# yinyunie/Pose2Room

Measured on AMD Instinct MI355X. Metric: P2RNet train-step samples/sec (T=1024,J=53,bs=32), higher is better.
Workload: dtype f32; 1 GPU; P2RNet full train step, bs=32/GPU, T=1024, J=53, seeds=512, proposals=128 (BASELINE configs[2]); input=P2RNet_dataloader over SyntheticPoseDataset, global_batch=32, frames=1024, parallelism=dp1

## Files before the change

include/p2r_hip.h:

```cpp
#ifndef P2R_HIP_H
#define P2R_HIP_H

#include <stdint.h>

#ifdef __cplusplus
extern "C" {
#endif

#define P2R_OK 0
#define P2R_EINVAL (-22)

int p2r_abi_version(void);
const char *p2r_build_arch(void);


int p2r_furthest_point_sampling(int b, int n, int m, const float *dataset,
                                float *temp, int *idxs, void *stream);

int p2r_gather_points(int b, int c, int n, int npoints, const float *points,
                      const int *idx, float *out, void *stream);

int p2r_gather_points_grad(int b, int c, int n, int npoints,
                           const float *grad_out, const int *idx,
                           float *grad_points, void *stream);

int p2r_ball_query(int b, int n, int m, float radius, int nsample,
                   const float *new_xyz, const float *xyz, int *idx,
                   void *stream);

int p2r_group_points(int b, int c, int n, int npoints, int nsample,
                     const float *points, const int *idx, float *out,
                     void *stream);

int p2r_group_points_grad(int b, int c, int n, int npoints, int nsample,
                          const float *grad_out, const int *idx,
                          float *grad_points, void *stream);

int p2r_three_nn(int b, int n, int m, const float *unknown, const float *known,
                 float *dist2, int *idx, void *stream);

int p2r_three_interpolate(int b, int c, int m, int n, const float *points,
                          const int *idx, const float *weight, float *out,
                          void *stream);

int p2r_three_interpolate_grad(int b, int c, int n, int m,
                               const float *grad_out, const int *idx,
                               const float *weight, float *grad_points,
                               void *stream);


#define P2R_NND_L2 0
#define P2R_NND_L1SMOOTH 1
#define P2R_NND_L1 2

int p2r_nn_distance(int B, int N, int M, int C, const float *pc1,
                    const float *pc2, int mode, float delta, float *dist1,
                    int64_t *idx1, float *dist2, int64_t *idx2, void *stream);

int p2r_nn_distance_grad(int B, int N, int M, int C, const float *pc1,
                         const float *pc2, int mode, float delta,
                         const int64_t *idx1, const int64_t *idx2,
                         const float *g1, const float *g2, float *grad_pc1,
                         float *grad_pc2, void *stream);


int p2r_det_loss_forward(int B, int S, int J, int T, int K, int G, int NC, int j0, float near_thr,
                         float far_thr, float w0, float w1, const float *seed_skeleton,
                         const float *vote_xyz, const int64_t *seed_inds, const float *vote_label,
                         const int64_t *vote_label_mask, const float *agg_xyz, const float *center,
                         const float *size, const double *heading, const float *obj_scores,
                         const float *sem_scores, const float *center_label, const float *box_mask,
                         const float *gt_size, const float *gt_heading, const int64_t *gt_cls,
                         float *partial, double *partial64, float *out32, double *out64, float *g_vote,
                         float *g_obj, float *g_c1, float *g_c2, float *g_size, double *g_head,
                         float *g_sem, void *stream);

int p2r_det_loss_backward(int B, int S, int K, int NC, const double *coef, const float *out32,
                          const float *g_vote, const float *g_obj, const float *g_c1, const float *g_c2,
                          const float *g_size, const double *g_head, const float *g_sem, float *d_vote,
                          float *d_obj, float *d_center, float *d_size, double *d_head, float *d_sem,
                          void *stream);


int p2r_nms3d(int B, int K, int stride, const double *boxes,
              const uint8_t *valid, double overlap_threshold, int old_type,
              int same_cls, uint8_t *keep, int *pick, int *npick, void *stream);


int p2r_stgcn_gcn_forward(int N, int T, int V, int K, const int *Lk_host,
                          const float *x, const float *W, const uint8_t *nbr,
                          const float *coef, const float *bias_cv, float *z,
                          float *stats_partial, void *stream);

int p2r_stgcn_gcn2_forward(int N, int T, int V, int K, int ltot, const float *x, const float *Wp,
                           const float *coef, const int *stream, int *stream_work,
                           const float *bias_cv, const float *addend, float *z, float *stats_partial,
                           int *n_partials, const float *bwd_u, const unsigned char *bwd_mask,
                           const float *bwd_fin, void *stream_h);

unsigned long long p2r_stgcn_gcn3_signature(int form);
int p2r_stgcn_gcn3_forward(int N, int T, int V, int K, int ltot, int form, const float *x, const float *Wp,
                           const float *coef, const float *bias_cv, const float *addend, float *z,
                           float *stats_partial, int *n_partials, const float *bwd_u,
                           const unsigned char *bwd_mask, const float *bwd_fin, void *stream_h);

int p2r_stgcn_gcn3_data_gradient_masked_addend(int N, int T, int V, int K, int ltot, const float *x,
                                               const float *Wp, const float *coef, const float *addend,
                                               const unsigned char *addend_mask, float *z, float *stats_partial,
                                               const float *bwd_u, const unsigned char *bwd_mask,
                                               const float *bwd_fin, void *stream_h);

int p2r_stgcn_gcn3_coef_grad(int N, int T, int V, int K, int ltot, const float *x, const float *dz,
                             const float *Wp, int n_blocks, float *dcoef_partial, void *stream);

int p2r_stgcn_gcn3_weight_grad(int N, int T, int V, int K, int ltot, const float *x, const float *dz,
                               const float *coef, int n_blocks, float *dw_partial, float *colsum_partial,
                               void *stream);

int p2r_stgcn_gcn_weight_grad(int N, int T, int V, int K, const int *Lk_host,
                              const float *x, const float *dz,
                              const uint8_t *nbr, const float *coef,
                              int n_blocks, float *dw_partial, float *colsum_partial,
                              int colsum_of_x, void *stream);

int p2r_stgcn_gcn_coef_grad(int N, int T, int V, int K, const int *Lk_host,
                            const float *x, const float *dz, const float *Wt,
                            const uint8_t *nbr, const float *coef, int n_blocks,
                            float *dcoef_partial, void *stream);


int p2r_bn_stats(int rows, int L, const float *x, float *partial, void *stream);

int p2r_bn_apply(int N, int C, int L, const float *x, const float *scale,
                 const float *shift, const float *res, int relu, float *y,
                 unsigned char *relu_mask, void *stream);

int p2r_bn_bwd_reduce(int N, int C, int L, const float *dy, const float *y,
                      const float *x, const float *mean, const float *invstd,
                      int relu, const float *mscale, const float *mshift,
                      float *partial, void *stream);

int p2r_bn_bwd_apply(int N, int C, int L, const float *dy, const float *y,
                     const float *x, const float *mean, const float *invstd,
                     const float *kscale, const float *m1, const float *m2,
                     int relu, const float *mscale, const float *mshift,
                     float *dx, float *dres, void *stream);

int p2r_bn_finalize(int P, int C, int width, const float *partial, double M, const float *gamma,
                    const float *beta, double eps, double momentum, float *running_mean,
                    float *running_var, long long *num_batches_tracked, float *out, void *stream);

int p2r_bn_bwd_finalize(int P, int C, const float *partial, double M, float *out, void *stream);


int p2r_stgcn_tconv_forward(int N, int T, int V, int taps, const float *x, const float *scale,
                            const float *shift, const float *W, const float *bias,
                            float *out, float *stats_partial, int *n_partials, void *stream);

int p2r_stgcn_tconv_weight_grad(int N, int T, int V, int taps, const float *x, const float *scale,
                                const float *shift, const float *dout, int n_blocks,
                                float *dw_partial, float *dbias_partial, void *stream);

int p2r_stgcn_tconv_weight_grad_dz(int N, int T, int V, int taps, const float *x, const float *fin,
                                   const float *dout, const float *dh, const float *m12, float *dz, int n_blocks,
                                   float *dw_partial, float *dbias_partial, void *stream);

int p2r_stgcn_tconv2_forward(int N, int T, int V, int taps, const float *x, const float *scale, const float *shift,
                             const float *Wp, const float *bias, float *out, float *stats_partial,
                             int *n_partials, const float *bwd_z, const float *bwd_fin, void *stream);

int p2r_stgcn_tconv3_forward(int N, int T, int V, int taps, const float *x, const float *scale, const float *shift,
                             const float *Wp, const float *bias, float *out, float *stats_partial,
                             int *n_partials, const float *bwd_z, const float *bwd_fin, void *stream);

int p2r_stgcn_tconv3_forward_add(int N, int T, int V, const float *x, const float *scale, const float *shift,
                                 const float *Wp, const float *bias, const float *add_ct, float *out, void *stream);


int p2r_embed3_forward(int N, int L, const float *x, const float *W, const float *bias,
                       float *out, void *stream);

int p2r_embed3_forward_stats(int N, int L, const float *x, const float *W, const float *bias,
                             float *out, float *scratch, float *stats, void *stream);

int p2r_embed3_weight_grad(int N, int L, const float *x, const float *dout, float *partial,
                           void *stream);

int p2r_embed3_weight_grad_lazy(int N, int L, const float *x, const float *g, const float *z, const float *coef,
                                float *partial, void *stream);

int p2r_embed_layer_backward(int N, int L, const float *g, const float *z, const float *coef, const float *zp,
                             const float *fin, const float *W, float *g_prev, float *sums, int n_blocks,
                             float *dw_part, float *db_part, void *stream);

int p2r_colsum(int rows, int T, int V, const float *x, float *out_partial, void *stream);

int p2r_sum_leading(int P, long long M, const float *in, float *out, int tr64, void *stream);


int p2r_sa_votes_forward(int b, int n, int m, int nsample, float radius, int C0,
                         int C1, int C2, const float *xyz, const float *new_xyz,
                         const float *features, const float *w1, const float *b1,
                         const float *w2, const float *b2, int *idx, float *out,
                         float *G, float *H, unsigned char *amax, void *stream);

int p2r_sa_votes_backward(int b, int m, int nsample, int C, const float *dout, const float *out,
                          const unsigned char *amax, const float *H, const float *w2t,
                          const float *w1t, float *dZ2, float *dZ1, float *dG, void *stream);

int p2r_gemm_nt_256(int nb, int L, int split, const float *A, const float *B, float *partial,
                    void *stream);


#define P2R_PW_MAX_JOBS 8

typedef struct p2r_pw_job {
  const float *x, *x2, *tr, *w, *bias, *mz, *mfin;
  float *out, *stats;
  int k, rows, x_ctot, x_nlc, tr_mode, tr_ld, w_t, out_ctot, out_nlc, epilogue, mz_ctot, mfin_ld;
} p2r_pw_job;

int p2r_pw_gemm(int njobs, const p2r_pw_job *jobs, int B, int L, void *stream);

typedef struct p2r_pw_wjob {
  const float *x, *x2, *tr, *y, *ytr;
  float *dw_part, *db_part;
  int rows, k, x_ctot, x_nlc, tr_mode, tr_ld, y_ctot, y_nlc, ytr_ld, split;
} p2r_pw_wjob;
int p2r_pw_wgrad(int njobs, const p2r_pw_wjob *jobs, int B, int L, void *stream);

typedef struct p2r_pw_bnjob {
  const float *part, *gamma, *beta;
  float *running_mean, *running_var, *fin;
  long long *num_batches_tracked;
  double eps, momentum;
  int P, C, fin_ld;
} p2r_pw_bnjob;
int p2r_pw_bn_finalize(int njobs, const p2r_pw_bnjob *jobs, void *stream);

typedef struct p2r_pw_bnbjob {
  const float *part, *fin;
  float *coef, *dgamma, *dbeta;
  double M;
  int P, C, fin_ld, coef_ld, train;
} p2r_pw_bnbjob;
int p2r_pw_bn_bwd_finalize(int njobs, const p2r_pw_bnbjob *jobs, void *stream);

typedef struct p2r_pw_rjob {
  const float *in;
  float *out;
  int P, M;
} p2r_pw_rjob;
#define P2R_PW_MAX_RJOBS 48
int p2r_pw_reduce(int njobs, const p2r_pw_rjob *jobs, void *stream);

typedef struct p2r_mix_head {
  const float *logit, *log_sigma;
  const void *mu, *eps, *dpred;
  void *pred, *dmu;
  float *pi, *dlogit, *dlog_sigma;
  int D, f64;
} p2r_mix_head;
#define P2R_MIX_MAX_HEADS 4
int p2r_mdn_mix_forward(int nheads, const p2r_mix_head *heads, int B, int G, int L, int logit_ctot, void *stream);
int p2r_mdn_mix_backward(int nheads, const p2r_mix_head *heads, int B, int G, int L, int logit_ctot, int dlogit_ctot,
                         void *stream);

typedef struct p2r_mdn_sample_head {
  const float *pi, *log_sigma;
  const void *mu;
  void *out;
  int D, f64, head_id;
} p2r_mdn_sample_head;
#define P2R_MDN_SAMPLE_MAX_HEADS 3
int p2r_mdn_sample(int nheads, const p2r_mdn_sample_head *heads, int B, int G, int L, int pi_ctot, int H,
                   const int *n_samples, unsigned long long seed, int h_offset, void *stream);

typedef struct p2r_sample_store {
  const float *joints, *votes;
  const long long *frame_offset;
  const int *n_frames;
  const double *floor_height, *box_center;
  const float *box_heading, *box_size, *box_mask;
  const long long *box_cls;
  long long n_frames_total;
  int n_samples, J, K;
} p2r_sample_store;
typedef struct p2r_batch_out {
  float *input_joints, *vote_label;
  long long *vote_label_mask;
  float *center_label, *size, *heading, *box_label_mask;
  long long *sem_cls_label;
} p2r_batch_out;
#define P2R_BOX_VARIANTS 9
int p2r_assemble_batch(const p2r_sample_store *store, int B, const long long *sel, const double *aug, int augment,
                       int use_height, int num_frames, const p2r_batch_out *out, void *stream);


int p2r_gather_frames(int b, int c, int t, int j, int s, const float *x, const long long *inds, float *out,
                      void *stream);
int p2r_gather_frames_grad(int b, int c, int t, int j, int s, const float *dout, const long long *inds, float *dx,
                           void *stream);
int p2r_rowsum_short(long long rows, int v_len, float scale, const float *x, float *out, void *stream);

int p2r_vote_finish(int b, int s, int C, const float *net, const float *seed_features, const float *hip,
                    float *vote_xyz, float *feat_ncl, float *inv_norm, void *stream);
int p2r_vote_finish_grad(int b, int s, int C, const float *d_xyz, const float *d_feat, const float *feat_ncl,
                         const float *inv_norm, float *d_net, float *d_sf, void *stream);

int p2r_nearest_prefix(int b, int t, int s, const float *cum, const float *target, long long *inds, void *stream);


int p2r_absmax_bits(long long n, const float *x, unsigned *amax_bits, void *stream);

int p2r_bn_bwd_apply_amax(int N, int C, int L, const float *dy, const unsigned char *mask, const float *x,
                          const float *mean, const float *invstd, const float *kscale, const float *m1,
                          const float *m2, float *dx, float *dres, unsigned *amax_bits, void *stream);
int p2r_bn_apply_amax(int N, int C, int L, const float *x, const float *scale, const float *shift, const float *res,
                      float *y, unsigned char *mask, unsigned *amax_bits, void *stream);
int p2r_stgcn_tconv_weight_grad_dz_amax(int N, int T, int V, int taps, const float *x, const float *fin,
                                        const float *dout, const float *dh, const float *m12, float *dz, int n_blocks,
                                        float *dw_partial, float *dbias_partial, unsigned *amax_bits, void *stream);

int p2r_stgcn_tconvh_forward(int N, int T, int V, const float *x, const float *scale, const float *shift,
                             const void *Wh, const float *winv, const float *bias, float *out, float *stats_partial,
                             int *n_partials, const float *bwd_z, const float *bwd_fin, const unsigned *x_amax,
                             void *stream);

unsigned long long p2r_stgcn_gcn3h_signature(int form);
int p2r_stgcn_gcn3h_pairs(int form, int *pairs);
int p2r_stgcn_gcn3h_forward(int N, int T, int V, int K, int ltot, const float *x, const void *Wh, const float *winv,
                            const float *coef, const float *bias_cv, float *z, float *stats_partial, int *n_partials,
                            const unsigned *x_amax, void *stream);
int p2r_stgcn_gcn3h_data_gradient(int N, int T, int V, int K, int ltot, const float *dz, const void *Wh,
                                  const float *winv, const float *coef, const float *addend,
                                  const unsigned char *addend_mask, float *dx, const unsigned *dz_amax, void *stream);

unsigned long long p2r_stgcn_gcn3h_weight_grad_signature(void);
int p2r_stgcn_gcn3h_weight_grad(int N, int T, int V, int K, int ltot, const float *x, const float *dz, const float *coef,
                                int n_blocks, float *dw_partial, float *dbias_partial, const unsigned *x_amax,
                                const unsigned *dz_amax, void *stream);

int p2r_stgcn_gcn3h_coef_grad(int N, int T, int V, int K, int ltot, const float *x, const float *dz, const void *Wd,
                              const float *winv, int n_blocks, float *dcoef_partial, const unsigned *x_amax,
                              void *stream);

#ifdef __cplusplus
}
#endif
#endif
```

pose2room_amd/p2rnet/modules/stgcn.py:

```python
import torch
import torch.nn as nn

from ..registers import MODULES
from .stgcn_layers import Graph, st_gcn_block
from .sub_modules import SingleConv


def _point_mlp(cin, width, cout):
    return nn.Sequential(SingleConv(cin, width, kernel_size=1, order='cbr', padding=0, ndim=1),
                         SingleConv(width, width, kernel_size=1, order='cbr', padding=0, ndim=1),
                         SingleConv(width, cout, kernel_size=1, order='c', padding=0, ndim=1))


@MODULES.register_module
class STGCN(nn.Module):
    def __init__(self, cfg, optim_spec=None):
        super().__init__()
        self.optim_spec = optim_spec

        self.graph = Graph(layout='virtualroom', strategy='spatial', max_hop=5)
        self.register_buffer('A', torch.tensor(self.graph.A, dtype=torch.float32, requires_grad=False))

        self.n_seeds = cfg.config['data']['num_seeds']
        self.origin_joint_id = cfg.dataset_config.origin_joint_id
        width, out_channels = 64, 256
        kernel_size = (3, self.A.size(0))
        self.knn = 20

        self.pos_embed = _point_mlp(3, 64, width)
        self.sk_feat = _point_mlp(3, 64, width)
        self.st_gcn_networks = nn.ModuleList(
            [st_gcn_block(width, 64, kernel_size, 1, residual=False)] +
            [st_gcn_block(64, 64, kernel_size, 1) for _ in range(5)])
        from ..gcn_op import GraphTables
        tables = GraphTables(self.graph.A)
        for i, blk in enumerate(self.st_gcn_networks):
            blk.gcn.tables = tables
            blk.chain_input = i > 0
        self.conv_joint = nn.Conv1d(cfg.dataset_config.joint_num * 64, out_channels, kernel_size=1)
        self.edge_importance = nn.ParameterList(
            [nn.Parameter(torch.ones(self.A.size())) for _ in self.st_gcn_networks])

        n_frames = cfg.config['data']['num_frames']
        if self.n_seeds >= n_frames:
            self.seed_inds = torch.round(torch.linspace(0, n_frames - 1, self.n_seeds)).long()
        else:
            self.seed_sampling = cfg.config['data']['seed_sampling']

    def _select_seeds(self, hip):
        n_batch, n_frames, _ = hip.shape
        device = hip.device
        if self.n_seeds >= n_frames:
            return self.seed_inds.repeat(n_batch, 1).to(device)
        if self.seed_sampling == 'random':
            inds = torch.argsort(torch.rand(size=(n_batch, n_frames)), dim=1)[:, :self.n_seeds]
            return torch.sort(inds, dim=1)[0].to(device)
        if self.seed_sampling == 'uniform':
            step = torch.norm(torch.diff(hip, dim=1), dim=2)
            cum = torch.cumsum(torch.cat([torch.zeros(size=(n_batch, 1), device=device), step], dim=1).double(),
                               dim=1).float()
            stride = cum[:, -1] / (self.n_seeds - 1)
            target = stride.unsqueeze(-1) * torch.arange(self.n_seeds, dtype=torch.float, device=device)
            if cum.is_cuda and cum.dtype == torch.float32 and n_frames <= 40000:
                from .. import seed_op
                return seed_op.nearest_prefix(cum, target)
            return torch.argmin(torch.abs(cum.unsqueeze(-1) - target.unsqueeze(1)), dim=1)
        raise NotImplementedError

    @staticmethod
    def _mlp(seq, x, inner, add_ct=None):
        from .. import bn_op, tconv_op, embed_op
        if embed_op.supported(seq, x, inner, add_ct):
            return embed_op.embed_mlp(seq, x, inner, add_ct)
        s0, s1, s2 = seq
        fused = (x.is_cuda and len(seq) == 3 and hasattr(s0, 'batchnorm') and hasattr(s1, 'batchnorm')
                 and not hasattr(s2, 'batchnorm') and tconv_op.supported_embed3(x, s0.conv)
                 and x.shape[2] % inner == 0 and inner <= 64)
        if fused:
            z0s = None
            if s0.batchnorm.training:
                z, z0s = tconv_op.embed3(x, s0.conv, want_stats=True)
            else:
                z = tconv_op.embed3(x, s0.conv)
            z = z.view(x.shape[0], 64, x.shape[2] // inner, inner)
            fused = tconv_op.supported_pointwise(z, s0.batchnorm, s1.conv) and \
                tconv_op.supported_pointwise(z, s1.batchnorm, s2.conv)
            if fused:
                if s1.batchnorm.training:
                    z, zs = tconv_op.bn_relu_tconv(z, s0.batchnorm, s1.conv, stats=z0s, want_stats=True)
                    z = tconv_op.bn_relu_tconv(z, s1.batchnorm, s2.conv, stats=zs, add_ct=add_ct)
                else:
                    z = tconv_op.bn_relu_tconv(z, s0.batchnorm, s1.conv)
                    z = tconv_op.bn_relu_tconv(z, s1.batchnorm, s2.conv, add_ct=add_ct)
                return z.view(x.shape[0], 64, x.shape[2])
        for stage in seq:
            if x.is_cuda and hasattr(stage, 'batchnorm') and hasattr(stage, 'ReLU') and \
                    bn_op.supported(x, stage.batchnorm):
                x = bn_op.fused_bn_act(stage.conv(x), stage.batchnorm, None, relu=True)
            else:
                x = stage(x)
        if add_ct is not None:
            x = (x.view(x.shape[0], x.shape[1], -1, inner) + add_ct.unsqueeze(-1)).view(x.shape)
        return x

    def embed(self, input_joints):
        n_batch, n_frames, n_joints, _ = input_joints.shape
        device = input_joints.device
        hip = input_joints[:, :, self.origin_joint_id]
        win = torch.arange(n_frames, device=device).unsqueeze(-1) + \
            torch.arange(-self.knn // 2, self.knn // 2, device=device).unsqueeze(0)
        win = win.clamp_(0, n_frames - 1)
        offs = hip[:, win] - hip.unsqueeze(2)
        pe = self._mlp(self.pos_embed, offs.reshape(n_batch, n_frames * self.knn, 3).transpose(1, 2).contiguous(), self.knn)
        from .. import seed_op
        pe = pe.view(n_batch, -1, n_frames, self.knn)
        fused = seed_op.short_rows_supported(pe)
        pe = seed_op.mean_last(pe) if fused else pe.mean(dim=3)
        rel = input_joints - input_joints[:, :, self.origin_joint_id:self.origin_joint_id + 1]
        sk = self._mlp(self.sk_feat, rel.reshape(n_batch, n_frames * n_joints, 3).transpose(1, 2).contiguous(), n_joints,
                       add_ct=pe)
        return sk.view(n_batch, -1, n_frames, n_joints)

    def forward(self, input_joints, end_points=None):
        end_points = {} if end_points is None else end_points
        n_batch, n_frames, n_joints, n_dim = input_joints.size()
        seed_inds = self._select_seeds(input_joints[:, :, self.origin_joint_id])

        x = self.embed(input_joints)
        blocks = self.st_gcn_networks
        tables = blocks[0].gcn.tables
        if tables is not None and tables.gen2 and all(b.chainable(x, self.A) for b in blocks):
            from ..gcn_op import prepare_chain
            for gcn, prep in zip(blocks, prepare_chain(blocks, self.A, self.edge_importance, tables, frames=x.shape[2])):
                x, _ = gcn(x, prep.Aeff, prepared=prep)
        else:
            for gcn, importance in zip(blocks, self.edge_importance):
                x, _ = gcn(x, self.A * importance)

        seed_skeleton = torch.gather(
            input_joints, 1, seed_inds[:, :, None, None].expand(n_batch, self.n_seeds, n_joints, n_dim))
        if self.n_seeds < n_frames:
            from .. import seed_op
            if seed_op.seed_rows_supported(x, seed_inds):
                rows = seed_op.seed_rows(x, seed_inds)
            else:
                rows = x.permute(0, 2, 1, 3)[torch.arange(n_batch, device=x.device)[:, None], seed_inds]
            seed_features = torch.nn.functional.linear(
                rows.reshape(n_batch, self.n_seeds, -1),
                self.conv_joint.weight.squeeze(-1), self.conv_joint.bias)
        else:
            x = x.transpose(2, 3).reshape(n_batch, -1, n_frames)
            seed_features = self.conv_joint(x).transpose(1, 2)
            seed_features = torch.gather(
                seed_features, 1, seed_inds.unsqueeze(-1).expand(n_batch, self.n_seeds, seed_features.size(-1)))
        end_points['seed_inds'] = seed_inds
        end_points['seed_skeleton'] = seed_skeleton[..., :3]
        end_points['seed_features'] = seed_features
        return end_points
```

pose2room_amd/p2rnet/modules/stgcn_layers.py:

```python
from collections import deque

import numpy as np
import torch
import torch.nn as nn

_VIRTUALROOM_BONES = [
    (0, 1), (1, 3), (3, 5), (5, 19), (0, 2), (2, 4), (4, 6), (6, 20), (0, 7), (7, 8), (8, 9),
    (9, 10), (10, 21), (10, 22), (8, 11), (11, 13), (13, 15), (15, 17), (8, 12), (12, 14),
    (14, 16), (16, 18), (17, 23), (23, 24), (24, 25), (17, 26), (26, 27), (27, 28), (17, 29),
    (29, 30), (30, 31), (17, 32), (32, 33), (33, 34), (17, 35), (35, 36), (36, 37), (18, 38),
    (38, 39), (39, 40), (18, 41), (41, 42), (42, 43), (18, 44), (44, 45), (45, 46), (18, 47),
    (47, 48), (48, 49), (18, 50), (50, 51), (51, 52)]

_LAYOUTS = {'virtualroom': dict(num_node=53, bones=_VIRTUALROOM_BONES, center=0)}


def hop_distance(num_node, edges, max_hop):
    nbr = [[] for _ in range(num_node)]
    for i, j in edges:
        if i != j:
            nbr[i].append(j)
            nbr[j].append(i)
    hop = np.full((num_node, num_node), np.inf)
    for s in range(num_node):
        hop[s, s] = 0
        dq = deque([s])
        while dq:
            u = dq.popleft()
            if hop[s, u] >= max_hop:
                continue
            for v in nbr[u]:
                if np.isinf(hop[s, v]):
                    hop[s, v] = hop[s, u] + 1
                    dq.append(v)
    return hop


class Graph:

    def __init__(self, layout='virtualroom', strategy='spatial', max_hop=5, dilation=1):
        if layout not in _LAYOUTS:
            raise ValueError("Do Not Exist This Layout.")
        spec = _LAYOUTS[layout]
        self.max_hop, self.dilation = max_hop, dilation
        self.num_node, self.center = spec['num_node'], spec['center']
        self.edge = [(i, i) for i in range(self.num_node)] + list(spec['bones'])
        self.hop_dis = hop_distance(self.num_node, self.edge, max_hop)
        self.A = self._adjacency(strategy)

    def _adjacency(self, strategy):
        V = self.num_node
        hops = list(range(0, self.max_hop + 1, self.dilation))
        reach = np.zeros((V, V))
        for h in hops:
            reach[self.hop_dis == h] = 1
        col = reach.sum(0)
        inv = np.zeros(V)
        inv[col > 0] = col[col > 0] ** (-1)
        norm = reach * inv[None, :]
        if strategy == 'uniform':
            return norm[None]
        if strategy == 'distance':
            return np.stack([np.where(self.hop_dis == h, norm, 0.0) for h in hops])
        if strategy == 'spatial':
            dc = self.hop_dis[:, self.center]
            same = dc[:, None] == dc[None, :]
            closer = dc[:, None] > dc[None, :]
            planes = []
            for h in hops:
                at_h = self.hop_dis == h
                root = np.where(at_h & same, norm, 0.0)
                close = np.where(at_h & closer, norm, 0.0)
                further = np.where(at_h & ~same & ~closer, norm, 0.0)
                if h == 0:
                    planes.append(root)
                else:
                    planes.append(root + close)
                    planes.append(further)
            return np.stack(planes)
        raise ValueError("Do Not Exist This Strategy")


class ConvTemporalGraphical(nn.Module):

    def __init__(self, in_channels, out_channels, kernel_size, t_kernel_size=1, t_stride=1,
                 t_padding=0, t_dilation=1, bias=True):
        super().__init__()
        self.kernel_size = kernel_size
        self.out_channels = out_channels
        self.tables = None
        self.fused = True
        self.conv = nn.Conv2d(in_channels, out_channels * kernel_size, kernel_size=(t_kernel_size, 1),
                              padding=(t_padding, 0), stride=(t_stride, 1), dilation=(t_dilation, 1),
                              bias=bias)

    def forward(self, x, A, want_stats=False, with_residual=False, bn_link=None, prepared=None, lazy_res=False):
        assert A.size(0) == self.kernel_size
        if self.tables is not None and self.fused:
            from .. import gcn_op
            if gcn_op.supported(x, self.conv.weight, A):
                return gcn_op.graph_conv(x, self.conv.weight, self.conv.bias, A, self.tables, want_stats,
                                         with_residual, bn_link, prepared, lazy_res), A
        assert not want_stats and not with_residual and prepared is None
        y = self.conv(x)
        n, kc, t, v = y.size()
        y = y.view(n, self.kernel_size, kc // self.kernel_size, t, v)
        z = torch.einsum('nkctv,kvw->nctw', (y, A))
        return z.contiguous(), A


def _zero(x):
    return 0


def _iden(x):
    return x


class st_gcn_block(nn.Module):

    def __init__(self, in_channels, out_channels, kernel_size, stride=1, dropout=0, residual=True):
        super().__init__()
        assert len(kernel_size) == 2 and kernel_size[0] % 2 == 1
        padding = ((kernel_size[0] - 1) // 2, 0)
        self.gcn = ConvTemporalGraphical(in_channels, out_channels, kernel_size[1])
        self.tcn = nn.Sequential(
            nn.BatchNorm2d(out_channels),
            nn.ReLU(inplace=True),
            nn.Conv2d(out_channels, out_channels, (kernel_size[0], 1), (stride, 1), padding),
            nn.BatchNorm2d(out_channels),
            nn.Dropout(dropout, inplace=True),
        )
        if not residual:
            self.residual = _zero
        elif in_channels == out_channels and stride == 1:
            self.residual = _iden
        else:
            self.residual = nn.Sequential(
                nn.Conv2d(in_channels, out_channels, kernel_size=1, stride=(stride, 1)),
                nn.BatchNorm2d(out_channels))
        self.relu = nn.ReLU(inplace=True)

    fused_bn = True
    fused_tconv = True
    lazy_residual_grad = True
    chain_input = False

    def chainable(self, x, A):
        if not (self.fused_bn and x.is_cuda and self.tcn[4].p == 0):
            return False
        from .. import bn_op, gcn_op, tconv_op
        return (self.training and self.fused_tconv and self.gcn.tables is not None and self.gcn.fused
                and gcn_op.supported(x, self.gcn.conv.weight, A) and bn_op.supported(x, self.tcn[0])
                and tconv_op.supported(x, self.tcn[0], self.tcn[2]))

    def forward(self, x, A, prepared=None):
        res = self.residual(x)
        if self.fused_bn and x.is_cuda and self.tcn[4].p == 0:
            from .. import bn_op, gcn_op, tconv_op
            chain = self.chainable(x, A)
            assert chain or prepared is None
            lazy = False
            if chain:
                if self.residual is _iden and x.requires_grad:
                    in_link = getattr(x, '_p2r_bn_link', None) if self.chain_input else None
                    lazy = self.lazy_residual_grad and self.tcn[3].training
                    (z, zstats, res), A = self.gcn(x, A, want_stats=True, with_residual=True, bn_link=in_link,
                                                   prepared=prepared, lazy_res=lazy)
                else:
                    (z, zstats), A = self.gcn(x, A, want_stats=True, prepared=prepared)
                wp = (prepared.tcn_wp_f, prepared.tcn_wp_b) if prepared is not None and z.shape[3] == 53 else None
                u, ustats = tconv_op.bn_relu_tconv(z, self.tcn[0], self.tcn[2], stats=zstats, want_stats=True, wp=wp)
                res_t = res if torch.is_tensor(res) else None
                return bn_op.fused_bn_act(u, self.tcn[3], res_t, relu=True, stats=ustats, link=bn_op.BNLink(),
                                          lazy_res=lazy), A
            x, A = self.gcn(x, A)
            if bn_op.supported(x, self.tcn[0]):
                if self.fused_tconv and tconv_op.supported(x, self.tcn[0], self.tcn[2]):
                    u = tconv_op.bn_relu_tconv(x, self.tcn[0], self.tcn[2])
                else:
                    h = bn_op.fused_bn_act(x, self.tcn[0], None, relu=True)
                    u = self.tcn[2](h)
                res_t = res if torch.is_tensor(res) else None
                return bn_op.fused_bn_act(u, self.tcn[3], res_t, relu=True), A
        else:
            x, A = self.gcn(x, A)
        x = self.tcn(x) + res
        return self.relu(x), A
```

pose2room_amd/p2rnet/seed_op.py:

```python
import ctypes

import torch
from torch.autograd import Function

from .. import _lib


def _rowsum(x, V, scale):
    out = torch.empty(x.shape[:-1], dtype=torch.float32, device=x.device)
    with torch.cuda.device(x.device):
        _lib.check(_lib.lib().p2r_rowsum_short(ctypes.c_longlong(x.numel() // V), V, ctypes.c_float(scale), _lib.ptr(x),
                                               _lib.ptr(out), _lib.current_stream(x.device)), "rowsum_short")
    return out


def short_rows_supported(x):
    return x.is_cuda and x.dtype == torch.float32 and 1 <= x.shape[-1] <= 64


class _SeedRows(Function):

    @staticmethod
    def forward(ctx, x, seed_inds):
        x = x.contiguous()
        inds = seed_inds.long().contiguous()
        B, C, T, J = x.shape
        S = inds.shape[1]
        out = torch.empty((B, S, C * J), dtype=torch.float32, device=x.device)
        with torch.cuda.device(x.device):
            _lib.check(_lib.lib().p2r_gather_frames(B, C, T, J, S, _lib.ptr(x), _lib.ptr(inds), _lib.ptr(out),
                                                    _lib.current_stream(x.device)), "gather_frames")
        ctx.save_for_backward(inds)
        ctx.dims = (B, C, T, J, S)
        return out

    @staticmethod
    def backward(ctx, dout):
        (inds,) = ctx.saved_tensors
        B, C, T, J, S = ctx.dims
        dout = dout.contiguous()
        dx = torch.empty((B, C, T, J), dtype=torch.float32, device=dout.device)
        with torch.cuda.device(dout.device):
            _lib.check(_lib.lib().p2r_gather_frames_grad(B, C, T, J, S, _lib.ptr(dout), _lib.ptr(inds), _lib.ptr(dx),
                                                         _lib.current_stream(dout.device)), "gather_frames_grad")
        return dx, None


def seed_rows_supported(x, seed_inds):
    return (x.is_cuda and x.dtype == torch.float32 and x.dim() == 4 and seed_inds.is_cuda and seed_inds.dim() == 2
            and seed_inds.dtype in (torch.int64, torch.int32) and seed_inds.shape[0] == x.shape[0])


def seed_rows(x, seed_inds):
    return _SeedRows.apply(x, seed_inds)


class _MeanLast(Function):

    @staticmethod
    def forward(ctx, x):
        x = x.contiguous()
        ctx.shape = x.shape
        return _rowsum(x, x.shape[-1], 1.0 / x.shape[-1])

    @staticmethod
    def backward(ctx, g):
        return (g * (1.0 / ctx.shape[-1])).unsqueeze(-1).expand(ctx.shape)


def mean_last(x):
    return _MeanLast.apply(x)


class _AddBroadcastLast(Function):

    @staticmethod
    def forward(ctx, a, b):
        ctx.V = a.shape[-1]
        return a + b.unsqueeze(-1)

    @staticmethod
    def backward(ctx, g):
        db = None
        if ctx.needs_input_grad[1]:
            gc = g.contiguous()
            db = _rowsum(gc, ctx.V, 1.0)
        return (g if ctx.needs_input_grad[0] else None), db


def add_broadcast_last(a, b):
    return _AddBroadcastLast.apply(a, b)


def nearest_prefix(cum, target):
    cum, target = cum.contiguous(), target.contiguous()
    B, T = cum.shape
    S = target.shape[1]
    out = torch.empty((B, S), dtype=torch.int64, device=cum.device)
    with torch.cuda.device(cum.device):
        _lib.check(_lib.lib().p2r_nearest_prefix(B, T, S, _lib.ptr(cum), _lib.ptr(target), _lib.ptr(out),
                                                 _lib.current_stream(cum.device)), "nearest_prefix")
    return out
```

Before: 798.6 samples/s.

## Fuse final ST-GCN block BN+residual+ReLU into seed-frame gather

```diff
diff --git a/include/p2r_hip.h b/include/p2r_hip.h
--- a/include/p2r_hip.h
+++ b/include/p2r_hip.h
@@ -311,6 +311,16 @@
 int p2r_nearest_prefix(int b, int t, int s, const float *cum, const float *target, long long *inds, void *stream);
 
 
+int p2r_seam_rows(int b, int c, int t, int j, int s, const float *z, const float *res, const float *scale,
+                  const float *shift, const long long *inds, float *rows, void *stream);
+int p2r_seam_sum_groups(int s);
+int p2r_seam_bwd_sums(int b, int c, int t, int j, int s, float *drows, const float *rows, const float *z,
+                      const long long *inds, const float *mean, const float *invstd, float *partial, void *stream);
+int p2r_seam_bwd_apply(int b, int c, int t, int j, int s, const float *g_rows, const float *z, const long long *inds,
+                       const float *mean, const float *invstd, const float *kscale, const float *m1, const float *m2,
+                       float *dz, float *dres, unsigned *amax_bits, void *stream);
+
+
 int p2r_absmax_bits(long long n, const float *x, unsigned *amax_bits, void *stream);
 
 int p2r_bn_bwd_apply_amax(int N, int C, int L, const float *dy, const unsigned char *mask, const float *x,
diff --git a/pose2room_amd/csrc/seed_seam.hip b/pose2room_amd/csrc/seed_seam.hip
--- /dev/null
+++ b/pose2room_amd/csrc/seed_seam.hip
@@ -0,0 +1,261 @@
+#include "p2r_common.h"
+
+namespace {
+
+constexpr int SS_THREADS = 256;
+constexpr int SS_SG = 4;
+constexpr int SS_MAXN = 4096;
+constexpr int SS_MAXI = SS_MAXN / SS_THREADS;
+
+__global__ __launch_bounds__(SS_THREADS) void seam_rows_kernel(int C, int T, int J, int S, const float *__restrict__ z,
+                                                               const float *__restrict__ res,
+                                                               const float *__restrict__ scale,
+                                                               const float *__restrict__ shift,
+                                                               const long long *__restrict__ inds,
+                                                               float *__restrict__ rows) {
+  const int b = blockIdx.x / S;
+  const long long t = inds[blockIdx.x];
+  const int n = C * J;
+  float *o = rows + (size_t)blockIdx.x * n;
+  if (t < 0 || t >= T) {
+    for (int e = threadIdx.x; e < n; e += SS_THREADS) o[e] = 0.f;
+    return;
+  }
+  const size_t fb = ((size_t)b * C * T + t) * J;
+  const float *zb = z + fb, *rb = res + fb;
+  const size_t plane = (size_t)T * J;
+  const int dc = SS_THREADS / J, dj = SS_THREADS - dc * J;
+  int c = threadIdx.x / J, j = threadIdx.x - c * J;
+  for (int e = threadIdx.x; e < n; e += SS_THREADS) {
+    const size_t a = (size_t)c * plane + j;
+    float v = fmaf(zb[a], scale[c], shift[c]);
+    v += rb[a];
+    o[e] = fmaxf(v, 0.f);
+    c += dc; j += dj;
+    if (j >= J) { j -= J; ++c; }
+  }
+}
+
+__global__ __launch_bounds__(SS_THREADS) void seam_bwd_sums_kernel(int C, int T, int J, int S, int groups,
+                                                                   float *__restrict__ drows,
+                                                                   const float *__restrict__ rows,
+                                                                   const float *__restrict__ z,
+                                                                   const long long *__restrict__ inds,
+                                                                   const float *__restrict__ mean,
+                                                                   const float *__restrict__ invstd,
+                                                                   float2 *__restrict__ partial) {
+  __shared__ float2 red[SS_MAXN];
+  const int b = blockIdx.x / groups, s0 = (blockIdx.x - b * groups) * SS_SG;
+  const int tid = threadIdx.x, n = C * J;
+  const size_t plane = (size_t)T * J;
+  float sg[SS_MAXI], sq[SS_MAXI], mu[SS_MAXI], is[SS_MAXI];
+  int zo[SS_MAXI];
+#pragma unroll
+  for (int i = 0; i < SS_MAXI; ++i) {
+    const int e = tid + SS_THREADS * i;
+    const int c = e < n ? e / J : 0;
+    sg[i] = 0.f; sq[i] = 0.f;
+    mu[i] = mean[c]; is[i] = invstd[c];
+    zo[i] = c * (int)plane + (e - c * J);
+  }
+  for (int s = s0; s < min(S, s0 + SS_SG); ++s) {
+    const long long t = inds[(size_t)b * S + s];
+    if (t < 0 || t >= T) continue;
+    float *dr = drows + ((size_t)b * S + s) * n;
+    const float *rr = rows + ((size_t)b * S + s) * n;
+    const float *zb = z + ((size_t)b * C * T + t) * J;
+    float d[SS_MAXI], r[SS_MAXI], zv[SS_MAXI];
+#pragma unroll
+    for (int i = 0; i < SS_MAXI; ++i) {
+      const int e = tid + SS_THREADS * i;
+      if (e < n) {
+        d[i] = __builtin_nontemporal_load(dr + e);
+        r[i] = __builtin_nontemporal_load(rr + e);
+        zv[i] = zb[zo[i]];
+      }
+    }
+#pragma unroll
+    for (int i = 0; i < SS_MAXI; ++i) {
+      const int e = tid + SS_THREADS * i;
+      if (e < n) {
+        const float g = r[i] > 0.f ? d[i] : 0.f;
+        dr[e] = g;
+        sg[i] += g;
+        sq[i] += g * ((zv[i] - mu[i]) * is[i]);
+      }
+    }
+  }
+#pragma unroll
+  for (int i = 0; i < SS_MAXI; ++i) {
+    const int e = tid + SS_THREADS * i;
+    if (e < n) red[e] = make_float2(sg[i], sq[i]);
+  }
+  __syncthreads();
+  for (int c = tid >> 2; c < C; c += SS_THREADS / 4) {
+    float a = 0.f, q = 0.f;
+    for (int j = tid & 3; j < J; j += 4) { a += red[c * J + j].x; q += red[c * J + j].y; }
+    a += __shfl_xor(a, 1, 64); q += __shfl_xor(q, 1, 64);
+    a += __shfl_xor(a, 2, 64); q += __shfl_xor(q, 2, 64);
+    if ((tid & 3) == 0) partial[(size_t)blockIdx.x * C + c] = make_float2(a, q);
+  }
+}
+
+constexpr int SA_TT = 8;
+constexpr int SA_MAXHIT = 16;
+constexpr int SA_K = SA_TT * 64 / 64;
+
+__device__ __forceinline__ unsigned sa_abs_bits(float v) { return __float_as_uint(v) & 0x7fffffffu; }
+
+template <bool RES, bool AMAX>
+__global__ __launch_bounds__(SS_THREADS) void seam_bwd_apply_kernel(int C, int T, int J, int S,
+                                                                    const float *__restrict__ g_rows,
+                                                                    const float *__restrict__ z,
+                                                                    const long long *__restrict__ inds,
+                                                                    const float *__restrict__ mean,
+                                                                    const float *__restrict__ invstd,
+                                                                    const float *__restrict__ kscale,
+                                                                    const float *__restrict__ m1,
+                                                                    const float *__restrict__ m2,
+                                                                    float *__restrict__ dz, float *__restrict__ dres,
+                                                                    unsigned *__restrict__ amax) {
+  __shared__ int hits[SA_TT][SA_MAXHIT];
+  __shared__ int nhit[SA_TT];
+  const int chunks = (T + SA_TT - 1) / SA_TT;
+  const int b = blockIdx.x / chunks, t0 = (blockIdx.x - b * chunks) * SA_TT;
+  const int tid = threadIdx.x, lane = tid & 63, wave = __builtin_amdgcn_readfirstlane(tid >> 6);
+  for (int f = 2 * wave; f < 2 * wave + 2; ++f) {
+    const long long t = t0 + f;
+    int cnt = 0;
+    const unsigned long long lt = lane == 0 ? 0ull : (~0ull >> (64 - lane));
+    for (int sb = 0; sb < S; sb += 64) {
+      const int s = sb + lane;
+      const bool hit = s < S && inds[(size_t)b * S + s] == t;
+      const unsigned long long m = __ballot(hit);
+      const int slot = cnt + (int)__builtin_popcountll(m & lt);
+      if (hit && slot < SA_MAXHIT) hits[f][slot] = s;
+      cnt += (int)__builtin_popcountll(m);
+    }
+    if (lane == 0) nhit[f] = cnt;
+  }
+  __syncthreads();
+  const int n = C * J, run = min(SA_TT, T - t0) * J;
+  const float *G = g_rows + (size_t)b * S * n;
+  int cnt[SA_K], o0[SA_K], o1[SA_K];
+  bool many = false;
+#pragma unroll
+  for (int k = 0; k < SA_K; ++k) {
+    const int e = lane + 64 * k;
+    cnt[k] = 0; o0[k] = 0; o1[k] = 0;
+    if (e < run) {
+      const int f = e / J, j = e - f * J;
+      cnt[k] = nhit[f];
+      o0[k] = (cnt[k] > 0 ? hits[f][0] : 0) * n + j;
+      o1[k] = (cnt[k] > 1 ? hits[f][1] : 0) * n + j;
+      many |= cnt[k] > 2;
+    }
+  }
+  unsigned am = 0;
+  const size_t plane = (size_t)T * J;
+  for (int c = wave; c < C; c += SS_THREADS / 64) {
+    const float mu = mean[c], is = invstd[c], kk = kscale[c], a1 = m1[c], a2 = m2[c];
+    const size_t base = ((size_t)b * C + c) * plane + (size_t)t0 * J;
+    auto finish = [&](int e, float zv, float g) {
+      const float xh = (zv - mu) * is;
+      const float o = kk * (g - a1 - xh * a2);
+      __builtin_nontemporal_store(o, dz + base + e);
+      if (AMAX) am = max(am, sa_abs_bits(o));
+      if (RES) __builtin_nontemporal_store(g, dres + base + e);
+    };
+    if (__builtin_expect(many, 0)) {
+#pragma unroll 1
+      for (int e = lane; e < run; e += 64) {
+        const int f = e / J, j = e - f * J, nh = nhit[f];
+        float acc = 0.f;
+        if (nh <= SA_MAXHIT) {
+          for (int i = 0; i < nh; ++i) acc += G[(size_t)hits[f][i] * n + c * J + j];
+        } else {
+          for (int s = 0; s < S; ++s)
+            if (inds[(size_t)b * S + s] == (long long)(t0 + f)) acc += G[(size_t)s * n + c * J + j];
+        }
+        finish(e, z[base + e], acc);
+      }
+      continue;
+    }
+    float zv[SA_K], g[SA_K];
+#pragma unroll
+    for (int k = 0; k < SA_K; ++k) {
+      const int e = lane + 64 * k;
+      g[k] = 0.f;
+      if (e < run) {
+        zv[k] = __builtin_nontemporal_load(z + base + e);
+        if (cnt[k] > 0) g[k] = G[o0[k] + c * J];
+        if (cnt[k] > 1) g[k] += G[o1[k] + c * J];
+      }
+    }
+#pragma unroll
+    for (int k = 0; k < SA_K; ++k) {
+      const int e = lane + 64 * k;
+      if (e < run) finish(e, zv[k], g[k]);
+    }
+  }
+  if (AMAX) {
+#pragma unroll
+    for (int off = 32; off >= 1; off >>= 1) am = max(am, (unsigned)__shfl_xor((int)am, off, 64));
+    if (lane == 0 && am != 0) atomicMax(amax, am);
+  }
+}
+
+bool seam_dims_ok(int b, int c, int t, int j, int s) {
+  return b >= 0 && c > 0 && t > 0 && j > 0 && j <= 64 && s >= 0 && (long long)c * j <= SS_MAXN &&
+         (long long)c * t * j < 0x7fffffffLL && (long long)s * c * j < 0x7fffffffLL &&
+         (long long)b * (s > t / SA_TT + 1 ? s : t / SA_TT + 1) < 0x7fffffffLL;
+}
+
+}
+
+extern "C" int p2r_seam_sum_groups(int s) { return s <= 0 ? 0 : (s + SS_SG - 1) / SS_SG; }
+
+extern "C" int p2r_seam_rows(int b, int c, int t, int j, int s, const float *z, const float *res, const float *scale,
+                             const float *shift, const long long *inds, float *rows, void *stream) {
+  if (!seam_dims_ok(b, c, t, j, s) || !res) return P2R_EINVAL;
+  if (b == 0 || s == 0) return P2R_OK;
+  hipLaunchKernelGGL(seam_rows_kernel, dim3((unsigned)(b * s)), dim3(SS_THREADS), 0, p2r_stream(stream), c, t, j, s, z, res,
+                     scale, shift, inds, rows);
+  P2R_LAUNCH_CHECK();
+  return P2R_OK;
+}
+
+extern "C" int p2r_seam_bwd_sums(int b, int c, int t, int j, int s, float *drows, const float *rows, const float *z,
+                                 const long long *inds, const float *mean, const float *invstd, float *partial,
+                                 void *stream) {
+  if (!seam_dims_ok(b, c, t, j, s) || s == 0) return P2R_EINVAL;
+  if (b == 0) return P2R_OK;
+  const int groups = p2r_seam_sum_groups(s);
+  hipLaunchKernelGGL(seam_bwd_sums_kernel, dim3((unsigned)(b * groups)), dim3(SS_THREADS), 0, p2r_stream(stream), c, t, j, s,
+                     groups, drows, rows, z, inds, mean, invstd, reinterpret_cast<float2 *>(partial));
+  P2R_LAUNCH_CHECK();
+  return P2R_OK;
+}
+
+extern "C" int p2r_seam_bwd_apply(int b, int c, int t, int j, int s, const float *g_rows, const float *z,
+                                  const long long *inds, const float *mean, const float *invstd, const float *kscale,
+                                  const float *m1, const float *m2, float *dz, float *dres, unsigned *amax_bits,
+                                  void *stream) {
+  if (!seam_dims_ok(b, c, t, j, s)) return P2R_EINVAL;
+  hipStream_t st = p2r_stream(stream);
+  if (amax_bits) {
+    hipError_t e = hipMemsetAsync(amax_bits, 0, sizeof(unsigned), st);
+    if (e != hipSuccess) return (int)e;
+  }
+  if (b == 0) return P2R_OK;
+  dim3 grid((unsigned)(b * ((t + SA_TT - 1) / SA_TT))), blk(SS_THREADS);
+#define P2R_SA(R, A) hipLaunchKernelGGL((seam_bwd_apply_kernel<R, A>), grid, blk, 0, st, c, t, j, s, g_rows, z, inds, mean, \
+                                        invstd, kscale, m1, m2, dz, dres, amax_bits)
+  if (dres && amax_bits) P2R_SA(true, true);
+  else if (dres) P2R_SA(true, false);
+  else if (amax_bits) P2R_SA(false, true);
+  else P2R_SA(false, false);
+#undef P2R_SA
+  P2R_LAUNCH_CHECK();
+  return P2R_OK;
+}
diff --git a/pose2room_amd/p2rnet/modules/stgcn.py b/pose2room_amd/p2rnet/modules/stgcn.py
--- a/pose2room_amd/p2rnet/modules/stgcn.py
+++ b/pose2room_amd/p2rnet/modules/stgcn.py
@@ -129,17 +129,31 @@
         x = self.embed(input_joints)
         blocks = self.st_gcn_networks
         tables = blocks[0].gcn.tables
+        seam = None
         if tables is not None and tables.gen2 and all(b.chainable(x, self.A) for b in blocks):
+            from .. import seed_op
             from ..gcn_op import prepare_chain
+            from .stgcn_layers import _iden
+            last = blocks[-1]
+            w_joint = self.conv_joint.weight.squeeze(-1)
+            defer = (self.n_seeds < n_frames and last.residual is _iden and last.tcn[3].training and x.requires_grad
+                     and seed_op.seed_seam_supported(x, x, seed_inds, w_joint))
             for gcn, prep in zip(blocks, prepare_chain(blocks, self.A, self.edge_importance, tables, frames=x.shape[2])):
-                x, _ = gcn(x, prep.Aeff, prepared=prep)
+                if defer and gcn is last:
+                    seam, _ = gcn(x, prep.Aeff, prepared=prep, defer_out=True)
+                else:
+                    x, _ = gcn(x, prep.Aeff, prepared=prep)
         else:
             for gcn, importance in zip(blocks, self.edge_importance):
                 x, _ = gcn(x, self.A * importance)
 
         seed_skeleton = torch.gather(
             input_joints, 1, seed_inds[:, :, None, None].expand(n_batch, self.n_seeds, n_joints, n_dim))
-        if self.n_seeds < n_frames:
+        if seam is not None:
+            u, ustats, res = seam
+            seed_features = seed_op.seed_seam(u, blocks[-1].tcn[3], res, ustats, seed_inds, w_joint,
+                                              self.conv_joint.bias)
+        elif self.n_seeds < n_frames:
             from .. import seed_op
             if seed_op.seed_rows_supported(x, seed_inds):
                 rows = seed_op.seed_rows(x, seed_inds)
diff --git a/pose2room_amd/p2rnet/modules/stgcn_layers.py b/pose2room_amd/p2rnet/modules/stgcn_layers.py
--- a/pose2room_amd/p2rnet/modules/stgcn_layers.py
+++ b/pose2room_amd/p2rnet/modules/stgcn_layers.py
@@ -154,17 +154,17 @@
                 and gcn_op.supported(x, self.gcn.conv.weight, A) and bn_op.supported(x, self.tcn[0])
                 and tconv_op.supported(x, self.tcn[0], self.tcn[2]))
 
-    def forward(self, x, A, prepared=None):
+    def forward(self, x, A, prepared=None, defer_out=False):
         res = self.residual(x)
         if self.fused_bn and x.is_cuda and self.tcn[4].p == 0:
             from .. import bn_op, gcn_op, tconv_op
             chain = self.chainable(x, A)
-            assert chain or prepared is None
+            assert chain or (prepared is None and not defer_out)
             lazy = False
             if chain:
                 if self.residual is _iden and x.requires_grad:
                     in_link = getattr(x, '_p2r_bn_link', None) if self.chain_input else None
-                    lazy = self.lazy_residual_grad and self.tcn[3].training
+                    lazy = self.lazy_residual_grad and self.tcn[3].training and not defer_out
                     (z, zstats, res), A = self.gcn(x, A, want_stats=True, with_residual=True, bn_link=in_link,
                                                    prepared=prepared, lazy_res=lazy)
                 else:
@@ -172,6 +172,9 @@
                 wp = (prepared.tcn_wp_f, prepared.tcn_wp_b) if prepared is not None and z.shape[3] == 53 else None
                 u, ustats = tconv_op.bn_relu_tconv(z, self.tcn[0], self.tcn[2], stats=zstats, want_stats=True, wp=wp)
                 res_t = res if torch.is_tensor(res) else None
+                if defer_out:
+                    assert res_t is not None
+                    return (u, ustats, res_t), A
                 return bn_op.fused_bn_act(u, self.tcn[3], res_t, relu=True, stats=ustats, link=bn_op.BNLink(),
                                           lazy_res=lazy), A
             x, A = self.gcn(x, A)
diff --git a/pose2room_amd/p2rnet/seed_op.py b/pose2room_amd/p2rnet/seed_op.py
--- a/pose2room_amd/p2rnet/seed_op.py
+++ b/pose2room_amd/p2rnet/seed_op.py
@@ -55,6 +55,74 @@
     return _SeedRows.apply(x, seed_inds)
 
 
+class _SeedSeam(Function):
+
+    @staticmethod
+    def forward(ctx, u, bn_weight, bn_bias, res, fin, seed_inds, weight, bias):
+        from . import math_mode
+        u, res = u.contiguous(), res.contiguous()
+        inds = seed_inds.long().contiguous()
+        B, C, T, J = u.shape
+        S = inds.shape[1]
+        rows = torch.empty((B * S, C * J), dtype=torch.float32, device=u.device)
+        with torch.cuda.device(u.device):
+            _lib.check(_lib.lib().p2r_seam_rows(B, C, T, J, S, _lib.ptr(u), _lib.ptr(res), _lib.ptr(fin[2]),
+                                                _lib.ptr(fin[3]), _lib.ptr(inds), _lib.ptr(rows),
+                                                _lib.current_stream(u.device)), "seam_rows")
+        out = torch.addmm(bias, rows, weight.t()) if bias is not None else rows @ weight.t()
+        ctx.save_for_backward(u, rows, fin, inds, weight)
+        ctx.dims = (B, C, T, J, S)
+        ctx.split = math_mode.split16()
+        ctx.has_bias = bias is not None
+        return out.view(B, S, -1)
+
+    @staticmethod
+    def backward(ctx, dout):
+        from . import bn_op, math_mode
+        u, rows, fin, inds, weight = ctx.saved_tensors
+        B, C, T, J, S = ctx.dims
+        dev = u.device
+        lib = _lib.lib()
+        d2 = dout.reshape(B * S, -1).contiguous()
+        dW = (rows.t() @ d2).t() if ctx.needs_input_grad[6] else None
+        dbias = d2.sum(0) if (ctx.has_bias and ctx.needs_input_grad[7]) else None
+        g = d2 @ weight
+        part = torch.empty((B * lib.p2r_seam_sum_groups(S), C, 2), dtype=torch.float32, device=dev)
+        with torch.cuda.device(dev):
+            st = _lib.current_stream(dev)
+            _lib.check(lib.p2r_seam_bwd_sums(B, C, T, J, S, _lib.ptr(g), _lib.ptr(rows), _lib.ptr(u), _lib.ptr(inds),
+                                             _lib.ptr(fin[0]), _lib.ptr(fin[1]), _lib.ptr(part), st), "seam_bwd_sums")
+        tot = bn_op.bwd_finalize(part, B * T * J)
+        dz = torch.empty_like(u)
+        dres = torch.empty_like(u) if ctx.needs_input_grad[3] else None
+        word = math_mode.new_word(dev) if ctx.split else None
+        with torch.cuda.device(dev):
+            _lib.check(lib.p2r_seam_bwd_apply(B, C, T, J, S, _lib.ptr(g), _lib.ptr(u), _lib.ptr(inds), _lib.ptr(fin[0]),
+                                              _lib.ptr(fin[1]), _lib.ptr(fin[2]), _lib.ptr(tot[2]), _lib.ptr(tot[3]),
+                                              _lib.ptr(dz), _lib.ptr(dres), _lib.ptr(word), st), "seam_bwd_apply")
+        if word is not None:
+            math_mode.announce(dz, word)
+        return dz, tot[1], tot[0], dres, None, None, dW, dbias
+
+
+def seed_seam_supported(u, res, seed_inds, weight):
+    return (u.is_cuda and u.dtype == torch.float32 and u.dim() == 4 and torch.is_tensor(res) and res.shape == u.shape
+            and res.dtype == torch.float32 and u.shape[1] * u.shape[3] <= 4096 and u.shape[3] <= 64
+            and u.shape[2] % 8 == 0 and u.numel() // max(u.shape[0], 1) < 2 ** 31
+            and seed_inds.is_cuda and seed_inds.dim() == 2 and seed_inds.shape[0] == u.shape[0]
+            and 0 < seed_inds.shape[1] and seed_inds.shape[1] * u.shape[1] * u.shape[3] < 2 ** 31
+            and seed_inds.dtype in (torch.int64, torch.int32)
+            and weight.dim() == 2 and weight.shape[1] == u.shape[1] * u.shape[3] and weight.dtype == torch.float32)
+
+
+def seed_seam(u, bn, res, stats, seed_inds, weight, bias):
+    from . import bn_op
+    fin = bn_op.finalize(stats, u.numel() // u.shape[1], bn)
+    if bn_op.GATE_HOOK is not None:
+        bn_op.GATE_HOOK(bn, u, fin[2], fin[3], res)
+    return _SeedSeam.apply(u, bn.weight, bn.bias, res, fin, seed_inds, weight, bias)
+
+
 class _MeanLast(Function):
 
     @staticmethod
```

Result: no change. 804.7 samples/s (median of 6 runs) (+0.8%).
